# zamazincode/cv-diffusion-model

Hardware: AMD Instinct MI355X
Metric: images/sec (whole node), 256×256 4-step LCM 'small'; PSNR vs CPU ref (higher is better)
Workload: dtype fp16

## Files before the change

cv-diffusion-model_amd/csrc/irbx.hip:

```cpp
#include <string>
#include <type_traits>
#include <vector>

#include "common.h"
#include "kernels.h"

namespace llie {

typedef uint32_t u32x2 __attribute__((ext_vector_type(2)));

typedef __bf16 bf16x2_t __attribute__((ext_vector_type(2)));
__device__ __forceinline__ float dot2_bf16(uint32_t a, uint32_t b, float c) {
  return __builtin_amdgcn_fdot2_f32_bf16(*reinterpret_cast<const bf16x2_t*>(&a), *reinterpret_cast<const bf16x2_t*>(&b), c, false);
}

template <typename T>
__device__ __forceinline__ typename Elem<T>::vec_t activate8(typename Elem<T>::vec_t v, const float* sc, const float* sh) {
  const u32x4 x = reinterpret_cast<const u32x4&>(v);
  const f32x4 s0 = *reinterpret_cast<const f32x4*>(sc), s1 = *reinterpret_cast<const f32x4*>(sc + 4);
  const f32x4 b0 = *reinterpret_cast<const f32x4*>(sh), b1 = *reinterpret_cast<const f32x4*>(sh + 4);
  u32x4 o;
  o[0] = act_clamp01_pack<T>(x[0], s0[0], s0[1], b0[0], b0[1]);
  o[1] = act_clamp01_pack<T>(x[1], s0[2], s0[3], b0[2], b0[3]);
  o[2] = act_clamp01_pack<T>(x[2], s1[0], s1[1], b1[0], b1[1]);
  o[3] = act_clamp01_pack<T>(x[3], s1[2], s1[3], b1[2], b1[3]);
  return reinterpret_cast<const typename Elem<T>::vec_t&>(o);
}

template <typename T, int KS, int NBW>
__global__ void __launch_bounds__(256, 2) expand_stats_kernel(const IrbxArgs a, const int RP) {
  constexpr int K = 16 * KS, XP = (K + 8) * 2;
  typedef typename Elem<T>::vec_t vec_t;
  __shared__ __align__(16) unsigned char sA[2][128 * XP];
  __shared__ __align__(16) float aff1[2][K];
  const int tid = threadIdx.x, lane = tid & 63, wave = tid >> 6;
  const int n = lane & 31, h = lane >> 5;
  const int b = blockIdx.z, tile = blockIdx.x;
  const int P = a.H * a.W;
  const T* x0 = reinterpret_cast<const T*>(a.x0) + (size_t)b * P * a.c0;
  const T* x1 = a.x1 ? reinterpret_cast<const T*>(a.x1) + (size_t)b * P * a.c1 : nullptr;
  const T* w1 = reinterpret_cast<const T*>(a.w1);

  vec_t wf[NBW][KS];
#pragma unroll
  for (int j = 0; j < NBW; ++j)
#pragma unroll
    for (int s = 0; s < KS; ++s) wf[j][s] = ld_vec<T>(w1 + (size_t)((wave * NBW + j) * 32 + n) * K + 16 * s + 8 * h);
  for (int i = tid; i < K; i += 256) {
    aff1[0][i] = a.as1[(size_t)b * K + i];
    aff1[1][i] = a.ab1[(size_t)b * K + i];
  }
  float s1[NBW], s2[NBW];
#pragma unroll
  for (int j = 0; j < NBW; ++j) s1[j] = s2[j] = 0.f;

  const int nsteps = RP / 128;
  const size_t p_first = (size_t)tile * RP;
  vec_t raw[KS];
  auto load = [&](int step) {
#pragma unroll
    for (int j = 0; j < KS; ++j) {
      const int v = tid + j * 256;
      const size_t pix = p_first + (size_t)step * 128 + v / (2 * KS);
      const int k = (v % (2 * KS)) * 8;
      raw[j] = k < a.c0 ? ld_vec<T>(x0 + pix * a.c0 + k) : ld_vec<T>(x1 + pix * a.c1 + (k - a.c0));
    }
  };
  load(0);
  wg_barrier();
  for (int step = 0; step < nsteps; ++step) {
    unsigned char* buf = sA[step & 1];
#pragma unroll
    for (int j = 0; j < KS; ++j) {
      const int v = tid + j * 256;
      const int k = (v % (2 * KS)) * 8;
      *reinterpret_cast<vec_t*>(buf + (v / (2 * KS)) * XP + k * 2) = activate8<T>(raw[j], &aff1[0][k], &aff1[1][k]);
    }
    if (step + 1 < nsteps) load(step + 1);
    wg_barrier();
#pragma unroll 1
    for (int pb = 0; pb < 4; ++pb) {
      vec_t af[KS];
#pragma unroll
      for (int s = 0; s < KS; ++s) af[s] = *reinterpret_cast<const vec_t*>(buf + (pb * 32 + n) * XP + (16 * s + 8 * h) * 2);
#pragma unroll
      for (int j = 0; j < NBW; ++j) {
        f32x16 acc;
#pragma unroll
        for (int r = 0; r < 16; ++r) acc[r] = 0.f;
#pragma unroll
        for (int s = 0; s < KS; ++s) acc = mfma16<T>(af[s], wf[j][s], acc);
        f32x2 t1 = {0.f, 0.f}, t2 = {0.f, 0.f};
#pragma unroll
        for (int r = 0; r < 16; r += 2) {
          const f32x2 v = {acc[r], acc[r + 1]};
          t1 += v;
          t2 = __builtin_elementwise_fma(v, v, t2);
        }
        s1[j] += t1[0] + t1[1];
        s2[j] += t2[0] + t2[1];
      }
    }
  }
  const int ntiles = P / RP;
#pragma unroll
  for (int j = 0; j < NBW; ++j) {
    s1[j] += __shfl_xor(s1[j], 32, 64);
    s2[j] += __shfl_xor(s2[j], 32, 64);
    if (h == 0) {
      const int c = (wave * NBW + j) * 32 + n;
      a.stats[((size_t)(b * ntiles + tile) * 2 + 0) * a.Chid + c] = 6.f * s1[j];
      a.stats[((size_t)(b * ntiles + tile) * 2 + 1) * a.Chid + c] = 36.f * s2[j];
    }
  }
}

constexpr int kXT_H = 8, kXT_W = 16;
constexpr int kXH_W = kXT_W + 2, kXH_H = kXT_H + 2;
constexpr int kXNPX = kXH_W * kXH_H;
constexpr int kXNPB = 6;

constexpr int SHP = 144;
constexpr int kXStamps = 9;

constexpr int kXDefaultVar = 0;
template <typename T, int KS, bool DBUF, bool STAMP = false, int ABL = 0, int DWV = 1, int VAR = kXDefaultVar>
__global__ void __launch_bounds__(256, (KS == 2 && !DBUF) ? 3 : 2) expand_dw_kernel(const IrbxArgs a, const int tiles_per_wg, const int chunks_per_wg) {
  constexpr int K = 16 * KS;
  constexpr int XP = (K + 8) * 2;
  constexpr int QSTEP = 256 / (2 * KS);
  constexpr int XTHR = QSTEP * 2 * KS;
  constexpr int XPT = (kXNPX + QSTEP - 1) / QSTEP;
  constexpr int SH_BYTES = kXNPB * 32 * SHP;
  constexpr bool PREF = KS <= 2;
  constexpr bool LATE = !PREF && (VAR & 1);
  constexpr bool NTST = (VAR & 2) != 0;
  typedef typename Elem<T>::vec_t vec_t;
  extern __shared__ __align__(16) unsigned char smem[];
  unsigned char* sH = smem;
  unsigned char* sX = smem + (DBUF ? 2 : 1) * SH_BYTES;
  T* wds = reinterpret_cast<T*>(sX + kXNPB * 32 * XP);
  float* aff2 = reinterpret_cast<float*>(wds + 10 * a.Chid);
  float* aff1 = aff2 + 2 * a.Chid;
  float* red = aff1 + 2 * K;
  constexpr bool PACC_LDS = KS <= 4;
  long long* pacc_lds = reinterpret_cast<long long*>(red + 2 * 256);
  long long pacc_reg[PACC_LDS ? 1 : KS];

  const int tid = threadIdx.x, lane = tid & 63, wave = tid >> 6;
  const int n = lane & 31, h = lane >> 5;
  const int chb = wave & 1, pxg = wave >> 1;
  const int b = blockIdx.z;
  const int tiles_x = a.W / kXT_W;
  const int P = a.H * a.W;
  const T* x0 = reinterpret_cast<const T*>(a.x0) + (size_t)b * P * a.c0;
  const T* x1 = a.x1 ? reinterpret_cast<const T*>(a.x1) + (size_t)b * P * a.c1 : nullptr;
  const T* w1 = reinterpret_cast<const T*>(a.w1);
  T* out = reinterpret_cast<T*>(a.out) + (size_t)b * P * a.Chid;
  const int chunk0 = blockIdx.y * chunks_per_wg;
  const int nchunks_all = a.Chid / 64;
  const int chunk1 = chunk0 + chunks_per_wg < nchunks_all ? chunk0 + chunks_per_wg : nchunks_all;

  if constexpr (DWV == 1) {
    for (int i = tid; i < 10 * a.Chid; i += 256) {
      const int t = i & 1, c = (i >> 1) % a.Chid, tap = 2 * ((i >> 1) / a.Chid) + t;
      wds[i] = tap < 9 ? (T)(6.f * a.wd[tap * a.Chid + c]) : (T)0.f;
    }
  } else {
    for (int i = tid; i < 9 * a.Chid; i += 256) wds[i] = (T)(6.f * a.wd[i]);
  }
  for (int i = tid; i < a.Chid; i += 256) {
    aff2[i] = a.as2[(size_t)b * a.Chid + i];
    aff2[a.Chid + i] = a.ab2[(size_t)b * a.Chid + i] * kSixth;
  }
  for (int i = tid; i < K; i += 256) {
    aff1[i] = a.as1[(size_t)b * K + i];
    aff1[K + i] = a.ab1[(size_t)b * K + i];
  }
  for (int i = tid; i < (kXNPB * 32 - kXNPX) * (XP / 16); i += 256)
    *reinterpret_cast<u32x4*>(sX + kXNPX * XP + i * 16) = u32x4{0u, 0u, 0u, 0u};

  uint32_t dmask[2][4];
#pragma unroll
  for (int s2 = 0; s2 < 2; ++s2)
#pragma unroll
    for (int d = 0; d < 4; ++d)
      dmask[s2][d] = ((n >> 3) == 2 * s2 + h && ((n & 7) >> 1) == d) ? ((n & 1) ? 0xFFFF0000u : 0x0000FFFFu) : 0u;
  int dq[2], drow[2];
#pragma unroll
  for (int blk = 0; blk < 2; ++blk) {
    drow[blk] = 2 * (2 * pxg + blk) + (n >> 4);
    dq[blk] = drow[blk] * kXH_W + (n & 15);
  }

  const int ntiles_img = tiles_x * (a.H / kXT_H);
  const int tile_first = tiles_per_wg > 0 ? blockIdx.x * tiles_per_wg : (int)(blockIdx.x * (unsigned)ntiles_img / gridDim.x);
  const int tile_end = tiles_per_wg > 0 ? tile_first + tiles_per_wg : (int)((blockIdx.x + 1) * (unsigned)ntiles_img / gridDim.x);
  const int tile_last = tile_end < ntiles_img ? tile_end : ntiles_img;

  const int xkv = tid % (2 * KS), xq0 = tid / (2 * KS), xk8 = xkv * 8;
  const bool xthr = XTHR == 256 || tid < XTHR;
  const bool xseg1 = xk8 >= a.c0;
  const T* xb = xseg1 ? x1 + (xk8 - a.c0) : x0 + xk8;
  const int xc = xseg1 ? a.c1 : a.c0;
  const bool xlast = xthr && (XPT - 1) * QSTEP + xq0 < kXNPX;
  int xrel[XPT];
#pragma unroll
  for (int j = 0; j < XPT; ++j) {
    const int q = xq0 + j * QSTEP;
    xrel[j] = (q / kXH_W - 1) * a.W + (q % kXH_W - 1);
  }
  unsigned char* sxw = sX + xq0 * XP + xk8 * 2;
  vec_t raw[XPT];
  auto load_tile = [&](int ty, int tx) {
    const int pix0 = ty * kXT_H * a.W + tx * kXT_W;
    const bool border = ty == 0 || tx == 0 || ty == a.H / kXT_H - 1 || tx == tiles_x - 1;
    if (!border) {
#pragma unroll
      for (int j = 0; j < XPT; ++j) {
        if (j < XPT - 1 ? xthr : xlast) raw[j] = ld_vec<T>(xb + (size_t)(pix0 + xrel[j]) * xc);
        else raw[j] = vec_t{};
      }
    } else {
#pragma unroll
      for (int j = 0; j < XPT; ++j) {
        const int q = xq0 + j * QSTEP;
        const int gy = ty * kXT_H - 1 + q / kXH_W, gx = tx * kXT_W - 1 + q % kXH_W;
        if ((j < XPT - 1 ? xthr : xlast) && gy >= 0 && gy < a.H && gx >= 0 && gx < a.W) raw[j] = ld_vec<T>(xb + (size_t)(pix0 + xrel[j]) * xc);
        else raw[j] = vec_t{};
      }
    }
  };
  int ty = tile_first / tiles_x, tx = tile_first % tiles_x;
  if ((PREF || LATE) && tile_first < tile_last) load_tile(ty, tx);
  vec_t wf[KS];
  auto load_wf = [&](int chunk) {
#pragma unroll
    for (int s = 0; s < KS; ++s) wf[s] = ld_vec<T>(w1 + (size_t)(chunk * 64 + chb * 32 + n) * K + 16 * s + 8 * h);
  };
  load_wf(chunk0);
  wg_barrier();

  unsigned long long tk[kXStamps] = {}, t_prev = 0;
  auto stamp = [&](int slot) {
    if constexpr (STAMP) {
      __builtin_amdgcn_sched_barrier(0);
      const unsigned long long now = __builtin_amdgcn_s_memtime();
      __builtin_amdgcn_sched_barrier(0);
      if (slot >= 0) tk[slot] += now - t_prev;
      t_prev = now;
    }
  };
  auto tile_barrier = [&]() {
    if constexpr (!(ABL & 32)) wg_barrier();
  };
  stamp(-1);
  const bool has_pool = a.pool != nullptr || a.pool_tot != nullptr;
  int par = 0;
  int pend_tile = -1, pend_chunk = 0, pend_par = 0;
  if constexpr (PACC_LDS) {
    if (tid < 64) {
#pragma unroll
      for (int q = 0; q < KS; ++q) pacc_lds[q * 64 + tid] = 0;
    }
  } else {
#pragma unroll
    for (int q = 0; q < KS; ++q) pacc_reg[q] = 0;
  }
  auto flush_pool = [&]() {
    if (pend_tile >= 0 && tid < 64) {
      const float* r = red + pend_par * 256;
      const int cbb = tid >> 5, ci = tid & 31;
      const float t = r[cbb * 64 + ci] + r[(cbb + 2) * 64 + ci];
      if (a.pool_tot) {
        const long long v = __float2ll_rn(t * kPoolFixScale);
        if constexpr (PACC_LDS) {
          pacc_lds[(pend_chunk - chunk0) * 64 + tid] += v;
        } else {
#pragma unroll
          for (int q = 0; q < KS; ++q) pacc_reg[q] += (pend_chunk - chunk0 == q) ? v : 0ll;
        }
      } else {
        a.pool[((size_t)b * ntiles_img + pend_tile) * a.Chid + pend_chunk * 64 + tid] = t;
      }
    }
    pend_tile = -1;
  };

  for (int tile = tile_first; tile < tile_last; ++tile) {
    const int y0 = ty * kXT_H, x0p = tx * kXT_W;
    int tyn = ty, txn = tx + 1;
    if (txn == tiles_x) { txn = 0; ++tyn; }
    if (!PREF && !LATE) load_tile(ty, tx);
    __builtin_amdgcn_s_waitcnt(0x0F70);
    stamp(0);
#pragma unroll
    for (int j = 0; j < XPT; ++j) {
      if (j < XPT - 1 ? xthr : xlast)
        *reinterpret_cast<vec_t*>(sxw + j * QSTEP * XP) = activate8<T>(raw[j], aff1 + xk8, aff1 + K + xk8);
    }
    stamp(1);
    if (PREF && tile + 1 < tile_last) load_tile(tyn, txn);
    const bool border = ty == 0 || tx == 0 || ty == a.H / kXT_H - 1 || tx == tiles_x - 1;
    bool ok[3] = {true, true, true};
    if (border) {
#pragma unroll
      for (int i = 0; i < 3; ++i) {
        const int q = (pxg * 3 + i) * 32 + n;
        const int gy = y0 - 1 + q / kXH_W, gx = x0p - 1 + q % kXH_W;
        ok[i] = q < kXNPX && gy >= 0 && gy < a.H && gx >= 0 && gx < a.W;
      }
    }
    stamp(2);
    tile_barrier();
    stamp(3);
    if (!DBUF) flush_pool();
    stamp(4);

    for (int chunk = chunk0; chunk < chunk1; ++chunk) {
      unsigned char* buf = sH + (DBUF ? par * SH_BYTES : 0);
      if (!DBUF && chunk > chunk0) {
        tile_barrier();
        flush_pool();
        stamp(5);
      }
      const int ch0 = chunk * 64 + chb * 32;
      f32x4 sc2[4], sh2[4];
#pragma unroll
      for (int g = 0; g < 4; ++g) {
        sc2[g] = *reinterpret_cast<const f32x4*>(aff2 + ch0 + 8 * g + 4 * h);
        sh2[g] = *reinterpret_cast<const f32x4*>(aff2 + a.Chid + ch0 + 8 * g + 4 * h);
      }
      constexpr int NACC = KS <= 2 ? 3 : 1;
      f32x16 accs[NACC];
      if constexpr (NACC == 3) {
#pragma unroll
        for (int i = 0; i < 3; ++i) {
          const int q = (pxg * 3 + i) * 32 + n;
#pragma unroll
          for (int r = 0; r < 16; ++r) accs[i][r] = 0.f;
#pragma unroll
          for (int s = 0; s < KS; ++s)
            accs[i] = mfma16<T>(wf[s], *reinterpret_cast<const vec_t*>(sX + q * XP + (16 * s + 8 * h) * 2), accs[i]);
        }
        load_wf(chunk + 1 < chunk1 ? chunk + 1 : chunk0);
      }
#pragma unroll
      for (int i = 0; i < 3; ++i) {
        const int q = (pxg * 3 + i) * 32 + n;
        if constexpr (NACC == 1) {
#pragma unroll
          for (int r = 0; r < 16; ++r) accs[0][r] = 0.f;
#pragma unroll
          for (int s = 0; s < KS; ++s)
            accs[0] = mfma16<T>(wf[s], *reinterpret_cast<const vec_t*>(sX + q * XP + (16 * s + 8 * h) * 2), accs[0]);
          if (i == 2) load_wf(chunk + 1 < chunk1 ? chunk + 1 : chunk0);
        }
        const f32x16 acc = accs[NACC == 3 ? i : 0];
        uint32_t pk[4][2];
#pragma unroll
        for (int g = 0; g < 4; ++g)
#pragma unroll
          for (int j = 0; j < 2; ++j)
            pk[g][j] = affine_clamp01_pack<T>(acc[4 * g + 2 * j], acc[4 * g + 2 * j + 1], sc2[g][2 * j], sc2[g][2 * j + 1],
                                              sh2[g][2 * j], sh2[g][2 * j + 1]);
        if (border) {
#pragma unroll
          for (int g = 0; g < 4; ++g)
#pragma unroll
            for (int j = 0; j < 2; ++j) pk[g][j] = ok[i] ? pk[g][j] : 0u;
        }
        u32x4 lo, hi2;
#pragma unroll
        for (int j = 0; j < 2; ++j) {
          const u32x2 r02 = __builtin_amdgcn_permlane32_swap(pk[0][j], pk[2][j], false, false);
          const u32x2 r13 = __builtin_amdgcn_permlane32_swap(pk[1][j], pk[3][j], false, false);
          lo[j] = r02[0]; lo[2 + j] = r02[1];
          hi2[j] = r13[0]; hi2[2 + j] = r13[1];
        }
        *reinterpret_cast<u32x4*>(buf + q * SHP + (chb * 4 + 2 * h) * 16) = lo;
        *reinterpret_cast<u32x4*>(buf + q * SHP + (chb * 4 + 2 * h + 1) * 16) = hi2;
      }
      stamp(6);
      tile_barrier();
      if (DBUF) flush_pool();
      if constexpr (LATE) {
        if (chunk + 1 == chunk1 && tile + 1 < tile_last) load_tile(tyn, txn);
      }
      stamp(7);
      if constexpr (DWV == 1) {
        typedef float f32x4v __attribute__((ext_vector_type(4)));
        const int li = lane & 15, g = lane >> 4;
        uint32_t amask[4];
#pragma unroll
        for (int d = 0; d < 4; ++d)
          amask[d] = (((li & 7) >> 1) == d && (g >> 1) == (li >> 3)) ? ((li & 1) ? 0xFFFF0000u : 0x0000FFFFu) : 0u;
        const uint32_t* wpair = reinterpret_cast<const uint32_t*>(wds) + chunk * 64 + chb * 32 + li;
        const uint32_t wsel = (g & 1) ? 0x03020302u : 0x01000100u;
        f32x4v dacc[2][4];
#pragma unroll
        for (int c2 = 0; c2 < 2; ++c2)
#pragma unroll
          for (int r = 0; r < 4; ++r) dacc[c2][r] = f32x4v{0.f, 0.f, 0.f, 0.f};
        const unsigned char* bbase = buf + ((4 * pxg) * kXH_W + li) * SHP + (chb * 4 + (g >> 1)) * 16;
        const bool upper = (g & 1) != 0;
        vec_t bf[2][4];
        uint32_t wq[2];
        auto ld_step = [&](int step, vec_t (&bb)[4], uint32_t& w2) {
          const int pr = step >> 1, c2 = step & 1;
          const int ta = 2 * pr, tb = 2 * pr + 1 < 9 ? 2 * pr + 1 : 8;
          const int offa = (ta / 3) * kXH_W + ta % 3, offb = (tb / 3) * kXH_W + tb % 3;
          const unsigned char* p0 = bbase + (upper ? offb : offa) * SHP + c2 * 32;
#pragma unroll
          for (int r = 0; r < 4; ++r) bb[r] = *reinterpret_cast<const vec_t*>(p0 + r * kXH_W * SHP);
          w2 = wpair[pr * a.Chid + 16 * c2];
        };
        ld_step(0, bf[0], wq[0]);
#pragma unroll
        for (int step = 0; step < 10; ++step) {
          if (step + 1 < 10) ld_step(step + 1, bf[(step + 1) & 1], wq[(step + 1) & 1]);
          __builtin_amdgcn_sched_barrier(0);
          const int c2 = step & 1;
          const uint32_t wdup = __builtin_amdgcn_perm(wq[step & 1], wq[step & 1], wsel);
          u32x4 t;
#pragma unroll
          for (int d = 0; d < 4; ++d) t[d] = wdup & amask[d];
          const vec_t af = reinterpret_cast<const vec_t&>(t);
#pragma unroll
          for (int r = 0; r < 4; ++r) {
            if constexpr (!(ABL & 8)) dacc[c2][r] = mfma16x16<T>(af, bf[step & 1][r], dacc[c2][r]);
            else asm volatile("" :: "v"(bf[step & 1][r]), "v"(af));
          }
        }
        const int choff = 8 * (g >> 1) + 16 * (g & 1);
#pragma unroll
        for (int r = 0; r < 4; ++r) {
          uint32_t p0[2], p1[2];
#pragma unroll
          for (int j = 0; j < 2; ++j) {
            typedef T t2 __attribute__((ext_vector_type(2)));
            t2 o0, o1;
            o0[0] = (T)dacc[0][r][2 * j]; o0[1] = (T)dacc[0][r][2 * j + 1];
            o1[0] = (T)dacc[1][r][2 * j]; o1[1] = (T)dacc[1][r][2 * j + 1];
            p0[j] = *reinterpret_cast<uint32_t*>(&o0);
            p1[j] = *reinterpret_cast<uint32_t*>(&o1);
          }
          const u32x2 s0 = __builtin_amdgcn_permlane16_swap(p0[0], p1[0], false, false);
          const u32x2 s1 = __builtin_amdgcn_permlane16_swap(p0[1], p1[1], false, false);
          const u32x4 v = {s0[0], s1[0], s0[1], s1[1]};
          const int orow = 4 * pxg + r;
          T* op = out + ((size_t)(y0 + orow) * a.W + x0p + li) * a.Chid + chunk * 64 + chb * 32 + choff;
          if constexpr ((ABL & 4) != 0) op = out + ((size_t)orow * a.W + x0p + li) * a.Chid + chunk * 64 + chb * 32 + choff;
          if constexpr (ABL & 1) asm volatile("" :: "v"(v));
          else if constexpr (NTST) __builtin_nontemporal_store(v, reinterpret_cast<u32x4*>(op));
          else *reinterpret_cast<u32x4*>(op) = v;
        }
        if (has_pool && !(ABL & 2)) {
          float v[8];
#pragma unroll
          for (int c2 = 0; c2 < 2; ++c2)
#pragma unroll
            for (int e = 0; e < 4; ++e) v[4 * c2 + e] = (dacc[c2][0][e] + dacc[c2][1][e]) + (dacc[c2][2][e] + dacc[c2][3][e]);
#define LLIE_DPP_STEP(ROR)                                                                                               \
  _Pragma("unroll") for (int i = 0; i < 8; ++i)                                                                          \
      asm volatile("v_add_f32_dpp %0, %0, %0 row_ror:" #ROR " row_mask:0xf bank_mask:0xf" : "+v"(v[i]));
          asm volatile("s_nop 1" : "+v"(v[0]), "+v"(v[1]), "+v"(v[2]), "+v"(v[3]), "+v"(v[4]), "+v"(v[5]), "+v"(v[6]), "+v"(v[7]));
          LLIE_DPP_STEP(8)
          LLIE_DPP_STEP(4)
          LLIE_DPP_STEP(2)
          LLIE_DPP_STEP(1)
#undef LLIE_DPP_STEP
          if (li == 0) {
            float* rp = red + (DBUF ? par : 0) * 256 + wave * 64 + 4 * g;
            *reinterpret_cast<f32x4*>(rp) = f32x4{v[0], v[1], v[2], v[3]};
            *reinterpret_cast<f32x4*>(rp + 16) = f32x4{v[4], v[5], v[6], v[7]};
          }
          pend_tile = tile; pend_chunk = chunk; pend_par = DBUF ? par : 0;
        }
      } else
      {
        const T* wcol = wds + chunk * 64 + chb * 32 + n;
        f32x16 dacc[2];
#pragma unroll
        for (int r = 0; r < 16; ++r) dacc[0][r] = dacc[1][r] = 0.f;
        uint32_t wv[9];
#pragma unroll
        for (int tap = 0; tap < 9; ++tap) wv[tap] = *reinterpret_cast<const uint16_t*>(wcol + tap * a.Chid);
        vec_t bf[2][4];
        auto ld_tap = [&](int tap, vec_t (&bb)[4]) {
          const int ky = tap / 3, kx = tap % 3;
#pragma unroll
          for (int blk = 0; blk < 2; ++blk)
#pragma unroll
            for (int s2 = 0; s2 < 2; ++s2)
              bb[blk * 2 + s2] = *reinterpret_cast<const vec_t*>(buf + (dq[blk] + ky * kXH_W + kx) * SHP + (chb * 4 + 2 * s2 + h) * 16);
        };
        ld_tap(0, bf[0]);
#pragma unroll
        for (int tap = 0; tap < 9; ++tap) {
          if (tap + 1 < 9) ld_tap(tap + 1, bf[(tap + 1) & 1]);
          __builtin_amdgcn_sched_barrier(0);
          const uint32_t wdup = wv[tap] | (wv[tap] << 16);
          vec_t af[2];
#pragma unroll
          for (int s2 = 0; s2 < 2; ++s2) {
            u32x4 t;
#pragma unroll
            for (int d = 0; d < 4; ++d) t[d] = wdup & dmask[s2][d];
            af[s2] = reinterpret_cast<const vec_t&>(t);
          }
#pragma unroll
          for (int blk = 0; blk < 2; ++blk)
#pragma unroll
            for (int s2 = 0; s2 < 2; ++s2) {
              const vec_t bv = bf[tap & 1][blk * 2 + s2];
              if constexpr (!(ABL & 8)) dacc[blk] = mfma16<T>(af[s2], bv, dacc[blk]);
              else asm volatile("" :: "v"(bv), "v"(af[s2]));
            }
        }
#pragma unroll
        for (int blk = 0; blk < 2; ++blk) {
          uint32_t pk[4][2];
#pragma unroll
          for (int g = 0; g < 4; ++g) {
            typedef T t2 __attribute__((ext_vector_type(2)));
#pragma unroll
            for (int j = 0; j < 2; ++j) {
              t2 o;
              o[0] = (T)dacc[blk][4 * g + 2 * j];
              o[1] = (T)dacc[blk][4 * g + 2 * j + 1];
              pk[g][j] = *reinterpret_cast<uint32_t*>(&o);
            }
          }
          u32x4 lo, hi2;
#pragma unroll
          for (int j = 0; j < 2; ++j) {
            const u32x2 r02 = __builtin_amdgcn_permlane32_swap(pk[0][j], pk[2][j], false, false);
            const u32x2 r13 = __builtin_amdgcn_permlane32_swap(pk[1][j], pk[3][j], false, false);
            lo[j] = r02[0]; lo[2 + j] = r02[1];
            hi2[j] = r13[0]; hi2[2 + j] = r13[1];
          }
          T* op = out + ((size_t)(y0 + drow[blk]) * a.W + x0p + (n & 15)) * a.Chid + chunk * 64 + chb * 32 + 16 * h;
          if constexpr ((ABL & 4) != 0)
            op = out + ((size_t)(drow[blk]) * a.W + x0p + (n & 15)) * a.Chid + chunk * 64 + chb * 32 + 16 * h;
          if constexpr ((ABL & 16) != 0) {
            T* cp = out + (((((size_t)tile * nchunks_all + chunk) * 4 + wave) * 2 + blk) * 1024) + lane * 8;
            *reinterpret_cast<u32x4*>(cp) = lo;
            *reinterpret_cast<u32x4*>(cp + 512) = hi2;
          } else if constexpr (!(ABL & 1)) {
            *reinterpret_cast<u32x4*>(op) = lo;
            *reinterpret_cast<u32x4*>(op + 8) = hi2;
          } else {
            asm volatile("" :: "v"(lo), "v"(hi2));
          }
        }
        if (has_pool && !(ABL & 2)) {
          float v[16];
#pragma unroll
          for (int r = 0; r < 16; ++r) v[r] = dacc[0][r] + dacc[1][r];
          {
            uint32_t m = (n & 16) ? 0xFFFFFFFFu : 0u;
            asm volatile("" : "+v"(m));
#pragma unroll
            for (int i = 0; i < 8; ++i) {
              const uint32_t lo = __float_as_uint(v[i]), hi = __float_as_uint(v[8 + i]);
              const float keep = __uint_as_float((hi & m) | (lo & ~m));
              const int send = (int)((lo & m) | (hi & ~m));
              v[i] = keep + __int_as_float(__builtin_amdgcn_ds_swizzle(send, 0x401F));
            }
            m = (n & 8) ? 0xFFFFFFFFu : 0u;
            asm volatile("" : "+v"(m));
#pragma unroll
            for (int i = 0; i < 4; ++i) {
              const uint32_t lo = __float_as_uint(v[i]), hi = __float_as_uint(v[4 + i]);
              const float keep = __uint_as_float((hi & m) | (lo & ~m));
              const int send = (int)((lo & m) | (hi & ~m));
              v[i] = keep + __int_as_float(__builtin_amdgcn_update_dpp(0, send, 0x128, 0xF, 0xF, false));
            }
          }
#pragma unroll
          for (int i = 0; i < 4; ++i) {
            v[i] += __int_as_float(__builtin_amdgcn_update_dpp(0, __float_as_int(v[i]), 0xB1, 0xF, 0xF, false));
            v[i] += __int_as_float(__builtin_amdgcn_update_dpp(0, __float_as_int(v[i]), 0x4E, 0xF, 0xF, false));
            v[i] += __int_as_float(__builtin_amdgcn_update_dpp(0, __float_as_int(v[i]), 0x141, 0xF, 0xF, false));
          }
          if ((n & 7) == 0) {
            f32x4 o = {v[0], v[1], v[2], v[3]};
            *reinterpret_cast<f32x4*>(red + (DBUF ? par : 0) * 256 + wave * 64 + 8 * (n >> 3) + 4 * h) = o;
          }
          pend_tile = tile; pend_chunk = chunk; pend_par = DBUF ? par : 0;
        }
      }
      if (DBUF) par ^= 1;
      stamp(8);
    }
    ty = tyn; tx = txn;
  }
  if constexpr (STAMP) {
    if (a.dbg && lane == 0) {
      const size_t wg = ((size_t)blockIdx.z * gridDim.y + blockIdx.y) * gridDim.x + blockIdx.x;
#pragma unroll
      for (int i = 0; i < kXStamps; ++i) a.dbg[(wg * 4 + wave) * kXStamps + i] = tk[i];
    }
  }
  if (has_pool) {
    wg_barrier();
    flush_pool();
    if (a.pool_tot && tid < 64) {
#pragma unroll
      for (int q = 0; q < KS; ++q)
        if (chunk0 + q < chunk1) atomicAdd(a.pool_tot + (size_t)b * a.Chid + (chunk0 + q) * 64 + tid, (unsigned long long)(PACC_LDS ? pacc_lds[q * 64 + tid] : pacc_reg[PACC_LDS ? 0 : q]));
    }
  }
}

int irbx_stats_rows(int P);
bool irbx_supported(int dtype, int Cin, int c0, int Chid, int H, int W) {
  if (dtype != 1 && dtype != 2) return false;
  if (Cin != 32 && Cin != 64 && Cin != 96) return false;
  if (c0 % 16 || Chid != 4 * Cin) return false;
  return W % kXT_W == 0 && H % kXT_H == 0 && (H * W) % irbx_stats_rows(H * W) == 0;
}
int irbx_pool_tiles(int H, int W) { return (H / kXT_H) * (W / kXT_W); }
int irbx_stats_rows(int P) {
  int rp = 128;
  while (rp < 1024 && rp * 2 * 64 <= P) rp *= 2;
  return rp;
}

static int g_irbx_dbuf = 0, g_irbx_tiles = 4, g_irbx_stamp = 0, g_irbx_ablate = 0, g_irbx_dwv = 1;
static int g_irbx_grid[3] = {0, 0, 0};
void irbx_grid(int ks, int v) {
  for (int i = 0; i < 3; ++i)
    if (ks == 0 || ks == 2 * (i + 1)) g_irbx_grid[i] = v;
}
static int g_irbx_var = kXDefaultVar;
void irbx_var(int v) { g_irbx_var = v; }
void irbx_dwv(int v) { g_irbx_dwv = v; }
void irbx_ablate(int v) { g_irbx_ablate = v; }
static unsigned long long* g_irbx_dbg = nullptr;
static size_t g_irbx_dbg_n = 0;
void irbx_stamp(int v) { g_irbx_stamp = v; }
hipError_t irbx_stamp_fetch(double* out) {
  if (!g_irbx_dbg || !g_irbx_dbg_n) return hipErrorInvalidValue;
  std::vector<unsigned long long> h(g_irbx_dbg_n);
  hipError_t e = hipMemcpy(h.data(), g_irbx_dbg, g_irbx_dbg_n * 8, hipMemcpyDeviceToHost);
  if (e != hipSuccess) return e;
  for (int i = 0; i < kXStamps; ++i) out[i] = 0.0;
  for (size_t i = 0; i < g_irbx_dbg_n; ++i) out[i % kXStamps] += (double)h[i];
  for (int i = 0; i < kXStamps; ++i) out[i] /= (double)(g_irbx_dbg_n / kXStamps);
  out[kXStamps] = (double)(g_irbx_dbg_n / kXStamps);
  return hipSuccess;
}
void irbx_tune(int dbuf, int tiles_per_wg) {
  if (dbuf >= 0) g_irbx_dbuf = dbuf;
  if (tiles_per_wg > 0) g_irbx_tiles = tiles_per_wg;
}

template <typename T, int KS, int NBW>
static hipError_t launch_stats_cfg(const IrbxArgs& a, hipStream_t s) {
  const int P = a.H * a.W, RP = irbx_stats_rows(P);
  static const std::string name = std::string("expand_stats_kernel<") + TypeName<T>::value + ", " + std::to_string(KS) + ", " +
                                  std::to_string(NBW) + ">";
  note_kernel(name.c_str());
  hipLaunchKernelGGL((expand_stats_kernel<T, KS, NBW>), dim3(P / RP, 1, a.B), dim3(256), 0, s, a, RP);
  return hipGetLastError();
}
template <typename T>
static hipError_t launch_stats_t(const IrbxArgs& a, hipStream_t s) {
  const int Cin = a.c0 + a.c1;
  if (Cin == 32 && a.Chid == 128) return launch_stats_cfg<T, 2, 1>(a, s);
  if (Cin == 64 && a.Chid == 256) return launch_stats_cfg<T, 4, 2>(a, s);
  if (Cin == 96 && a.Chid == 384) return launch_stats_cfg<T, 6, 3>(a, s);
  return hipErrorInvalidValue;
}
hipError_t launch_expand_stats(int dtype, const IrbxArgs& a, hipStream_t s) {
  if (!irbx_supported(dtype, a.c0 + a.c1, a.c0, a.Chid, a.H, a.W) || (a.c1 && !a.x1) || !a.stats) return hipErrorInvalidValue;
  if (a.Chid != 4 * (a.c0 + a.c1)) return hipErrorInvalidValue;
  return dtype == 1 ? launch_stats_t<half_t>(a, s) : launch_stats_t<bf16_t>(a, s);
}

template <typename T, int KS, bool DBUF>
static hipError_t launch_dw_cfg(const IrbxArgs& a, hipStream_t s) {
  const size_t lds = (size_t)(DBUF ? 2 : 1) * kXNPB * 32 * SHP + (size_t)kXNPB * 32 * (16 * KS + 8) * 2 + (size_t)10 * a.Chid * 2 +
                     (size_t)2 * a.Chid * 4 + (size_t)2 * 16 * KS * 4 + 2 * 256 * 4 + (KS <= 4 ? (size_t)KS * 64 * 8 : 0);
  static std::atomic<uint64_t> attr_done{0};
  if (hipError_t e = ensure_max_lds(reinterpret_cast<const void*>(&expand_dw_kernel<T, KS, DBUF>), 128 * 1024, attr_done); e != hipSuccess)
    return e;
  const int ntiles = irbx_pool_tiles(a.H, a.W), nchunks = a.Chid / 64;
  int tpw = g_irbx_tiles;
  while (tpw > 1 && ((a.W / kXT_W) % tpw || (long)(ntiles / tpw) * a.B < 2048)) tpw >>= 1;
  int cpw = nchunks;
  while (cpw > 1 && (long)(ntiles / tpw) * a.B * (nchunks / cpw) < 1024 && cpw % 2 == 0) cpw >>= 1;
  static const std::string name = std::string("expand_dw_kernel<") + TypeName<T>::value + ", " + std::to_string(KS) + ", " +
                                  (DBUF ? "1" : "0") + ">";
  note_kernel(name.c_str());
  dim3 grid(ntiles / tpw, nchunks / cpw, a.B);
  if (g_irbx_grid[KS / 2 - 1] > 0) {
    int gx = g_irbx_grid[KS / 2 - 1] / (a.B * (nchunks / cpw));
    gx = gx < 1 ? 1 : (gx > ntiles ? ntiles : gx);
    grid.x = gx;
    tpw = 0;
  }
  if constexpr (std::is_same<T, half_t>::value && !DBUF) {
    if (g_irbx_stamp || a.ablate) {
      IrbxArgs b = a;
      if (g_irbx_stamp) {
        const size_t n = (size_t)grid.x * grid.y * grid.z * 4 * kXStamps;
        if (n > g_irbx_dbg_n || !g_irbx_dbg) {
          if (g_irbx_dbg) (void)hipFree(g_irbx_dbg);
          hipError_t e = hipMalloc(reinterpret_cast<void**>(&g_irbx_dbg), n * 8);
          if (e != hipSuccess) return e;
        }
        g_irbx_dbg_n = n;
        b.dbg = g_irbx_dbg;
      }
      auto go = [&](auto kern) -> hipError_t {
        hipError_t e = hipFuncSetAttribute(reinterpret_cast<const void*>(kern), hipFuncAttributeMaxDynamicSharedMemorySize, 128 * 1024);
        if (e != hipSuccess) return e;
        hipLaunchKernelGGL(kern, grid, dim3(256), lds, s, b, tpw, cpw);
        return hipGetLastError();
      };
      if (g_irbx_stamp) {
        switch (a.ablate) {
          case 0: return go(&expand_dw_kernel<T, KS, DBUF, true, 0>);
          case 1: return go(&expand_dw_kernel<T, KS, DBUF, true, 1>);
          case 32: return go(&expand_dw_kernel<T, KS, DBUF, true, 32>);
        }
      } else {
        switch (a.ablate) {
          case 1: return go(&expand_dw_kernel<T, KS, DBUF, false, 1>);
          case 4: return go(&expand_dw_kernel<T, KS, DBUF, false, 4>);
          case 8: return go(&expand_dw_kernel<T, KS, DBUF, false, 8>);
          case 32: return go(&expand_dw_kernel<T, KS, DBUF, false, 32>);
          case 33: return go(&expand_dw_kernel<T, KS, DBUF, false, 33>);
        }
      }
      return hipErrorInvalidValue;
    }
  }
  if (g_irbx_dwv == 0) {
    static std::atomic<uint64_t> attr0{0};
    if (hipError_t e = ensure_max_lds(reinterpret_cast<const void*>(&expand_dw_kernel<T, KS, DBUF, false, 0, 0>), 128 * 1024, attr0); e != hipSuccess)
      return e;
    hipLaunchKernelGGL((expand_dw_kernel<T, KS, DBUF, false, 0, 0>), grid, dim3(256), lds, s, a, tpw, cpw);
    return hipGetLastError();
  }
  if constexpr (!DBUF) {
    if (g_irbx_var != kXDefaultVar || a.nt) {
      auto go = [&](auto kern) -> hipError_t {
        hipError_t e = hipFuncSetAttribute(reinterpret_cast<const void*>(kern), hipFuncAttributeMaxDynamicSharedMemorySize, 128 * 1024);
        if (e != hipSuccess) return e;
        hipLaunchKernelGGL(kern, grid, dim3(256), lds, s, a, tpw, cpw);
        return hipGetLastError();
      };
      switch (g_irbx_var | (a.nt ? 2 : 0)) {
        case 0: return go(&expand_dw_kernel<T, KS, DBUF, false, 0, 1, 0>);
        case 1: return go(&expand_dw_kernel<T, KS, DBUF, false, 0, 1, 1>);
        case 2: return go(&expand_dw_kernel<T, KS, DBUF, false, 0, 1, 2>);
        case 3: return go(&expand_dw_kernel<T, KS, DBUF, false, 0, 1, 3>);
      }
      return hipErrorInvalidValue;
    }
  }
  hipLaunchKernelGGL((expand_dw_kernel<T, KS, DBUF>), grid, dim3(256), lds, s, a, tpw, cpw);
  return hipGetLastError();
}
template <typename T>
static hipError_t launch_dw_t(const IrbxArgs& a, hipStream_t s) {
  const int Cin = a.c0 + a.c1;
  if (g_irbx_dbuf) {
    switch (Cin) {
      case 32: return launch_dw_cfg<T, 2, true>(a, s);
      case 64: return launch_dw_cfg<T, 4, false>(a, s);
      case 96: return launch_dw_cfg<T, 6, false>(a, s);
    }
  } else {
    switch (Cin) {
      case 32: return launch_dw_cfg<T, 2, false>(a, s);
      case 64: return launch_dw_cfg<T, 4, false>(a, s);
      case 96: return launch_dw_cfg<T, 6, false>(a, s);
    }
  }
  return hipErrorInvalidValue;
}
hipError_t launch_expand_dw(int dtype, const IrbxArgs& a0, hipStream_t s) {
  if (!irbx_supported(dtype, a0.c0 + a0.c1, a0.c0, a0.Chid, a0.H, a0.W) || (a0.c1 && !a0.x1) || !a0.out) return hipErrorInvalidValue;
  IrbxArgs a = a0;
  a.ablate = g_irbx_ablate;
  return dtype == 1 ? launch_dw_t<half_t>(a, s) : launch_dw_t<bf16_t>(a, s);
}

}
```

Before: 1044.

## Reuse halo-row B fragments across depthwise taps in MFMA expand kernel

Adds a DWV=2 depthwise path and makes it the default. The nine 3x3 taps are regrouped into per-column tap sets, and each B fragment loaded from LDS for a halo row feeds several output rows' MFMAs. Before, every tap pair reloaded four rows. The goal is fewer LDS reads per MFMA. In exchange it uses more registers (6 B fragments double-buffered), permutes the output pixel column mapping, and reorders the weight packing.

```diff
diff --git a/cv-diffusion-model_amd/csrc/irbx.hip b/cv-diffusion-model_amd/csrc/irbx.hip
--- a/cv-diffusion-model_amd/csrc/irbx.hip
+++ b/cv-diffusion-model_amd/csrc/irbx.hip
@@ -124,7 +124,7 @@
 constexpr int kXStamps = 9;
 
 constexpr int kXDefaultVar = 0;
-template <typename T, int KS, bool DBUF, bool STAMP = false, int ABL = 0, int DWV = 1, int VAR = kXDefaultVar>
+template <typename T, int KS, bool DBUF, bool STAMP = false, int ABL = 0, int DWV = 2, int VAR = kXDefaultVar>
 __global__ void __launch_bounds__(256, (KS == 2 && !DBUF) ? 3 : 2) expand_dw_kernel(const IrbxArgs a, const int tiles_per_wg, const int chunks_per_wg) {
   constexpr int K = 16 * KS;
   constexpr int XP = (K + 8) * 2;
@@ -161,9 +161,10 @@
   const int nchunks_all = a.Chid / 64;
   const int chunk1 = chunk0 + chunks_per_wg < nchunks_all ? chunk0 + chunks_per_wg : nchunks_all;
 
-  if constexpr (DWV == 1) {
+  if constexpr (DWV >= 1) {
     for (int i = tid; i < 10 * a.Chid; i += 256) {
-      const int t = i & 1, c = (i >> 1) % a.Chid, tap = 2 * ((i >> 1) / a.Chid) + t;
+      const int t = i & 1, c = (i >> 1) % a.Chid, p = (i >> 1) / a.Chid;
+      const int tap = DWV == 1 ? 2 * p + t : (p < 3 ? 3 * p + 2 * t : (p == 3 ? 1 + 3 * t : 7 + 2 * t));
       wds[i] = tap < 9 ? (T)(6.f * a.wd[tap * a.Chid + c]) : (T)0.f;
     }
   } else {
@@ -388,48 +389,88 @@
         if (chunk + 1 == chunk1 && tile + 1 < tile_last) load_tile(tyn, txn);
       }
       stamp(7);
-      if constexpr (DWV == 1) {
+      if constexpr (DWV >= 1) {
         typedef float f32x4v __attribute__((ext_vector_type(4)));
         const int li = lane & 15, g = lane >> 4;
+        const int pcol = DWV == 2 ? 2 * ((li + 4) & 7) + (((li + 4) >> 3) & 1) : li;
         uint32_t amask[4];
 #pragma unroll
         for (int d = 0; d < 4; ++d)
           amask[d] = (((li & 7) >> 1) == d && (g >> 1) == (li >> 3)) ? ((li & 1) ? 0xFFFF0000u : 0x0000FFFFu) : 0u;
         const uint32_t* wpair = reinterpret_cast<const uint32_t*>(wds) + chunk * 64 + chb * 32 + li;
         const uint32_t wsel = (g & 1) ? 0x03020302u : 0x01000100u;
+        auto afrag = [&](uint32_t w2) {
+          const uint32_t wdup = __builtin_amdgcn_perm(w2, w2, wsel);
+          u32x4 t;
+#pragma unroll
+          for (int d = 0; d < 4; ++d) t[d] = wdup & amask[d];
+          return reinterpret_cast<const vec_t&>(t);
+        };
         f32x4v dacc[2][4];
 #pragma unroll
         for (int c2 = 0; c2 < 2; ++c2)
 #pragma unroll
           for (int r = 0; r < 4; ++r) dacc[c2][r] = f32x4v{0.f, 0.f, 0.f, 0.f};
-        const unsigned char* bbase = buf + ((4 * pxg) * kXH_W + li) * SHP + (chb * 4 + (g >> 1)) * 16;
+        const unsigned char* bbase = buf + ((4 * pxg) * kXH_W + pcol) * SHP + (chb * 4 + (g >> 1)) * 16;
         const bool upper = (g & 1) != 0;
-        vec_t bf[2][4];
-        uint32_t wq[2];
-        auto ld_step = [&](int step, vec_t (&bb)[4], uint32_t& w2) {
-          const int pr = step >> 1, c2 = step & 1;
-          const int ta = 2 * pr, tb = 2 * pr + 1 < 9 ? 2 * pr + 1 : 8;
-          const int offa = (ta / 3) * kXH_W + ta % 3, offb = (tb / 3) * kXH_W + tb % 3;
-          const unsigned char* p0 = bbase + (upper ? offb : offa) * SHP + c2 * 32;
-#pragma unroll
-          for (int r = 0; r < 4; ++r) bb[r] = *reinterpret_cast<const vec_t*>(p0 + r * kXH_W * SHP);
-          w2 = wpair[pr * a.Chid + 16 * c2];
-        };
-        ld_step(0, bf[0], wq[0]);
-#pragma unroll
-        for (int step = 0; step < 10; ++step) {
-          if (step + 1 < 10) ld_step(step + 1, bf[(step + 1) & 1], wq[(step + 1) & 1]);
-          __builtin_amdgcn_sched_barrier(0);
-          const int c2 = step & 1;
-          const uint32_t wdup = __builtin_amdgcn_perm(wq[step & 1], wq[step & 1], wsel);
-          u32x4 t;
-#pragma unroll
-          for (int d = 0; d < 4; ++d) t[d] = wdup & amask[d];
-          const vec_t af = reinterpret_cast<const vec_t&>(t);
-#pragma unroll
-          for (int r = 0; r < 4; ++r) {
-            if constexpr (!(ABL & 8)) dacc[c2][r] = mfma16x16<T>(af, bf[step & 1][r], dacc[c2][r]);
-            else asm volatile("" :: "v"(bf[step & 1][r]), "v"(af));
+        if constexpr (DWV == 1) {
+          vec_t bf[2][4];
+          uint32_t wq[2];
+          auto ld_step = [&](int step, vec_t (&bb)[4], uint32_t& w2) {
+            const int pr = step >> 1, c2 = step & 1;
+            const int ta = 2 * pr, tb = 2 * pr + 1 < 9 ? 2 * pr + 1 : 8;
+            const int offa = (ta / 3) * kXH_W + ta % 3, offb = (tb / 3) * kXH_W + tb % 3;
+            const unsigned char* p0 = bbase + (upper ? offb : offa) * SHP + c2 * 32;
+#pragma unroll
+            for (int r = 0; r < 4; ++r) bb[r] = *reinterpret_cast<const vec_t*>(p0 + r * kXH_W * SHP);
+            w2 = wpair[pr * a.Chid + 16 * c2];
+          };
+          ld_step(0, bf[0], wq[0]);
+#pragma unroll
+          for (int step = 0; step < 10; ++step) {
+            if (step + 1 < 10) ld_step(step + 1, bf[(step + 1) & 1], wq[(step + 1) & 1]);
+            __builtin_amdgcn_sched_barrier(0);
+            const int c2 = step & 1;
+            const vec_t af = afrag(wq[step & 1]);
+#pragma unroll
+            for (int r = 0; r < 4; ++r) {
+              if constexpr (!(ABL & 8)) dacc[c2][r] = mfma16x16<T>(af, bf[step & 1][r], dacc[c2][r]);
+              else asm volatile("" :: "v"(bf[step & 1][r]), "v"(af));
+            }
+          }
+        } else {
+          vec_t bf[2][6];
+          auto ld_it = [&](int it, vec_t (&bb)[6]) {
+            const int c2 = it >> 1;
+#pragma unroll
+            for (int hr = 0; hr < 6; ++hr) {
+              const int off = (it & 1) ? ((upper && hr < 5) ? hr + 1 : hr) * kXH_W + 1 : hr * kXH_W + (upper ? 2 : 0);
+              bb[hr] = *reinterpret_cast<const vec_t*>(bbase + off * SHP + c2 * 32);
+            }
+          };
+          ld_it(0, bf[0]);
+#pragma unroll
+          for (int it = 0; it < 4; ++it) {
+            const int c2 = it >> 1, kind = it & 1;
+            uint32_t wq[3];
+#pragma unroll
+            for (int j = 0; j < 3 - kind; ++j) wq[j] = wpair[(3 * kind + j) * a.Chid + 16 * c2];
+            if (it + 1 < 4) ld_it(it + 1, bf[(it + 1) & 1]);
+            __builtin_amdgcn_sched_barrier(0);
+            vec_t af[3];
+#pragma unroll
+            for (int j = 0; j < 3 - kind; ++j) af[j] = afrag(wq[j]);
+#pragma unroll
+            for (int hr = 0; hr < 6; ++hr) {
+              const vec_t bv = bf[it & 1][hr];
+#pragma unroll
+              for (int r = 0; r < 4; ++r) {
+                const int j = kind == 0 ? hr - r : (hr == r ? 0 : (hr - r == 2 ? 1 : -1));
+                if (j < 0 || j > 2) continue;
+                if constexpr (!(ABL & 8)) dacc[c2][r] = mfma16x16<T>(af[j], bv, dacc[c2][r]);
+                else asm volatile("" :: "v"(bv), "v"(af[j]));
+              }
+            }
           }
         }
         const int choff = 8 * (g >> 1) + 16 * (g & 1);
@@ -449,8 +490,8 @@
           const u32x2 s1 = __builtin_amdgcn_permlane16_swap(p0[1], p1[1], false, false);
           const u32x4 v = {s0[0], s1[0], s0[1], s1[1]};
           const int orow = 4 * pxg + r;
-          T* op = out + ((size_t)(y0 + orow) * a.W + x0p + li) * a.Chid + chunk * 64 + chb * 32 + choff;
-          if constexpr ((ABL & 4) != 0) op = out + ((size_t)orow * a.W + x0p + li) * a.Chid + chunk * 64 + chb * 32 + choff;
+          T* op = out + ((size_t)(y0 + orow) * a.W + x0p + pcol) * a.Chid + chunk * 64 + chb * 32 + choff;
+          if constexpr ((ABL & 4) != 0) op = out + ((size_t)orow * a.W + x0p + pcol) * a.Chid + chunk * 64 + chb * 32 + choff;
           if constexpr (ABL & 1) asm volatile("" :: "v"(v));
           else if constexpr (NTST) __builtin_nontemporal_store(v, reinterpret_cast<u32x4*>(op));
           else *reinterpret_cast<u32x4*>(op) = v;
@@ -628,7 +669,7 @@
   return rp;
 }
 
-static int g_irbx_dbuf = 0, g_irbx_tiles = 4, g_irbx_stamp = 0, g_irbx_ablate = 0, g_irbx_dwv = 1;
+static int g_irbx_dbuf = 0, g_irbx_tiles = 4, g_irbx_stamp = 0, g_irbx_ablate = 0, g_irbx_dwv = 2;
 static int g_irbx_grid[3] = {0, 0, 0};
 void irbx_grid(int ks, int v) {
   for (int i = 0; i < 3; ++i)
@@ -678,6 +719,23 @@
   if (!irbx_supported(dtype, a.c0 + a.c1, a.c0, a.Chid, a.H, a.W) || (a.c1 && !a.x1) || !a.stats) return hipErrorInvalidValue;
   if (a.Chid != 4 * (a.c0 + a.c1)) return hipErrorInvalidValue;
   return dtype == 1 ? launch_stats_t<half_t>(a, s) : launch_stats_t<bf16_t>(a, s);
+}
+
+template <typename T, int KS, int DWV>
+static hipError_t launch_dw_var(const IrbxArgs& a, hipStream_t s, dim3 grid, size_t lds, int tpw, int cpw) {
+  auto go = [&](auto kern) -> hipError_t {
+    hipError_t e = hipFuncSetAttribute(reinterpret_cast<const void*>(kern), hipFuncAttributeMaxDynamicSharedMemorySize, 128 * 1024);
+    if (e != hipSuccess) return e;
+    hipLaunchKernelGGL(kern, grid, dim3(256), lds, s, a, tpw, cpw);
+    return hipGetLastError();
+  };
+  switch (g_irbx_var | (a.nt ? 2 : 0)) {
+    case 0: return go(&expand_dw_kernel<T, KS, false, false, 0, DWV, 0>);
+    case 1: return go(&expand_dw_kernel<T, KS, false, false, 0, DWV, 1>);
+    case 2: return go(&expand_dw_kernel<T, KS, false, false, 0, DWV, 2>);
+    case 3: return go(&expand_dw_kernel<T, KS, false, false, 0, DWV, 3>);
+  }
+  return hipErrorInvalidValue;
 }
 
 template <typename T, int KS, bool DBUF>
@@ -746,22 +804,18 @@
     hipLaunchKernelGGL((expand_dw_kernel<T, KS, DBUF, false, 0, 0>), grid, dim3(256), lds, s, a, tpw, cpw);
     return hipGetLastError();
   }
+  if (g_irbx_dwv == 1) {
+    if constexpr (!DBUF) {
+      if (g_irbx_var != kXDefaultVar || a.nt) return launch_dw_var<T, KS, 1>(a, s, grid, lds, tpw, cpw);
+    }
+    static std::atomic<uint64_t> attr1{0};
+    if (hipError_t e = ensure_max_lds(reinterpret_cast<const void*>(&expand_dw_kernel<T, KS, DBUF, false, 0, 1>), 128 * 1024, attr1); e != hipSuccess)
+      return e;
+    hipLaunchKernelGGL((expand_dw_kernel<T, KS, DBUF, false, 0, 1>), grid, dim3(256), lds, s, a, tpw, cpw);
+    return hipGetLastError();
+  }
   if constexpr (!DBUF) {
-    if (g_irbx_var != kXDefaultVar || a.nt) {
-      auto go = [&](auto kern) -> hipError_t {
-        hipError_t e = hipFuncSetAttribute(reinterpret_cast<const void*>(kern), hipFuncAttributeMaxDynamicSharedMemorySize, 128 * 1024);
-        if (e != hipSuccess) return e;
-        hipLaunchKernelGGL(kern, grid, dim3(256), lds, s, a, tpw, cpw);
-        return hipGetLastError();
-      };
-      switch (g_irbx_var | (a.nt ? 2 : 0)) {
-        case 0: return go(&expand_dw_kernel<T, KS, DBUF, false, 0, 1, 0>);
-        case 1: return go(&expand_dw_kernel<T, KS, DBUF, false, 0, 1, 1>);
-        case 2: return go(&expand_dw_kernel<T, KS, DBUF, false, 0, 1, 2>);
-        case 3: return go(&expand_dw_kernel<T, KS, DBUF, false, 0, 1, 3>);
-      }
-      return hipErrorInvalidValue;
-    }
+    if (g_irbx_var != kXDefaultVar || a.nt) return launch_dw_var<T, KS, 2>(a, s, grid, lds, tpw, cpw);
   }
   hipLaunchKernelGGL((expand_dw_kernel<T, KS, DBUF>), grid, dim3(256), lds, s, a, tpw, cpw);
   return hipGetLastError();
```

New measurement: 1048, median of 6. No clear change (+0.3%).
